# cleinc/bts

Measured on NVIDIA H100. Metric: training images/sec (352x704, DenseNet-161), higher is better.
Workload: dtype f32

## Files before the change

bts_b200/_lib.py:

```python
import ctypes
import glob
import os
import subprocess

_HERE = os.path.dirname(os.path.abspath(__file__))
_ROOT = os.path.dirname(_HERE)
LIB_PATH = os.path.join(_HERE, "libbts_b200.so")
CSRC = os.path.join(_HERE, "csrc")

NVCC_FLAGS = ["-gencode", "arch=compute_90a,code=sm_90a", "-lineinfo", "-O3", "-std=c++17",
              "-Xcompiler", "-fPIC", "--expt-relaxed-constexpr"]


def sources():
    return sorted(glob.glob(os.path.join(CSRC, "*.cu")))


def needs_build():
    if not os.path.isfile(LIB_PATH):
        return True
    t = os.path.getmtime(LIB_PATH)
    deps = sources() + glob.glob(os.path.join(CSRC, "*.cuh")) + glob.glob(os.path.join(_ROOT, "include", "*.h"))
    return any(os.path.getmtime(f) > t for f in deps)

# ... 29 lines not shown
_ll = ctypes.c_longlong

SIGNATURES = {
    "bts_version": [ctypes.c_char_p, _i],
    "bts_lpg_fwd": [_p, _p, _i, _i, _i, _i, _i, _p],
    "bts_lpg_fwd_fused": [_p, _p, _p, _p, _f, _i, _i, _i, _i, _i, _i, _p],
    "bts_lpg_bwd": [_p, _p, _p, _i, _i, _i, _i, _i, _i, _p],
    "bts_lpg_bwd_fused": [_p, _p, _p, _f, _i, _p, _p, _i, _i, _i, _i, _i, _i, _p],
    "bts_lpg_fwd_h": [_p, _p, _i, _i, _i, _i, _i],
    "bts_lpg_bwd_h": [_p, _p, _p, _i, _i, _i, _i, _i, _i],
    "bts_silog_fwd": [_p, _p, _p, _ll, _f, _p, _p, _p],
    "bts_silog_bwd": [_p, _p, _p, _ll, _f, _p, _p, _p, _p],
    "bts_plane_head_fwd": [_p, _p, _p, _p, _f, _i, _i, _i, _i, _i, _p],
    "bts_plane_head_bwd": [_p, _p, _p, _p, _f, _i, _i, _i, _i, _i, _p],
    "bts_conv_n_tile": [_i],
    "bts_conv_packed_floats": [_i, _i, _i, _i],
    "bts_conv_pack_weights": [_p, _ll, _ll, _ll, _ll, _i, _i, _i, _i, _i, _p, _p],
    "bts_conv_fwd": [_p, _ll, _i, _i, _i, _i, _i, _i, _i, _i, _i, _i, _p, _i, _p, _p, _i, _p, _ll, _i, _i, _p],
    "bts_conv_fwd_stats": [_p, _ll, _i, _i, _i, _i, _i, _i, _i, _i, _i, _i, _p, _i, _p, _p, _i, _p, _ll, _i, _i, _p, _p, _p],
    "bts_conv_fwd_ex": [_p, _ll, _i, _i, _i, _i, _i, _i, _i, _i, _i, _i, _i, _i, _i, _p, _i, _p, _p, _i, _p, _ll, _i, _i, _p,
                        _p, _p],
    "bts_conv_fwd_bnbwd": [_p, _ll, _i, _i, _i, _i, _i, _i, _i, _i, _i, _i, _i, _i, _i, _p, _i, _p, _ll, _i, _p, _ll, _p, _i,
                           _p, _p, _p],
    "bts_bn_bwd_coef": [_p, _p, _ll, _i, _p, _p, _p, _p, _p],
    "bts_conv_group_window": [_i, _i],
    "bts_conv_packed_floats_grouped": [_i, _i, _i, _i],
    "bts_conv_group_n_tile": [_i],
    "bts_conv_pack_weights_grouped": [_p, _ll, _ll, _ll, _ll, _i, _i, _i, _i, _i, _p, _p],
    "bts_conv_wgrad_grouped_plan": [_i, _i, _i, _i, _i, _i, _i, _p, _p],
    "bts_conv_wgrad_grouped": [_p, _ll, _i, _i, _i, _i, _i, _i, _i, _i, _i, _i, _p, _ll, _p, _i, _p, _ll, _ll, _ll, _ll, _i, _p],
    "bts_conv_wgrad_plan": [_i, _i, _i, _i, _i, _i, _i, _i, _p, _p],
    "bts_conv_wgrad": [_p, _ll, _i, _i, _i, _i, _i, _i, _i, _i, _i, _i, _p, _p, _i, _p, _ll, _i, _p, _i, _p, _ll, _ll,
                       _ll, _ll, _i, _p],
    "bts_conv_c1_workspace_floats": [_i, _i],
    "bts_conv_c1_fwd": [_p, _ll, _i, _i, _i, _i, _i, _p, _ll, _ll, _ll, _i, _p, _p],
    "bts_conv_c1_dgrad": [_p, _p, _i, _i, _i, _i, _i, _p, _ll, _ll, _ll, _p, _ll, _p],
    "bts_conv_c1_wgrad": [_p, _ll, _p, _p, _i, _i, _i, _i, _i, _p, _p, _ll, _ll, _ll, _p],
    "bts_bn_stats": [_p, _ll, _ll, _i, _p, _p, _p],
    "bts_bn_finalize": [_p, _p, _ll, _i, _p, _p, _f, _f, _p, _p, _p, _p, _p, _p, _p],
    "bts_bn_finalize_track": [_p, _p, _ll, _i, _p, _p, _f, _f, _p, _p, _p, _p, _p, _p, _p, _p],
    "bts_bn_fold": [_i, _p, _p, _f, _p, _p, _p, _p, _p, _p, _p],
    "bts_bn_relu_bwd_reduce": [_p, _ll, _p, _ll, _ll, _i, _p, _p, _p, _p, _p, _p, _p, _p],
    "bts_bn_relu_bwd_apply": [_p, _ll, _p, _ll, _ll, _i, _p, _p, _p, _p, _ll, _i, _p],
    "bts_wgrad2_set_tma": [_i],
    "bts_wgrad2_set_min_pixels": [_ll],
    "bts_wgrad2_set_min_kblocks": [_i],
# ... 68 lines not shown
```

bts_b200/conv.py:

```python
import ctypes
import weakref

import torch

from . import _lib
from .ops import _need_cuda, _ptr, _stream

ACT = {None: 0, "none": 0, "elu": 1, "sigmoid": 2}
import os as _os

PW_FWD = _os.environ.get("BTS_B200_PW_FWD", "1") == "1"
PW_WGRAD = True
PW_MIN_PIXELS = 200000
TRACE = _os.environ.get("BTS_B200_TRACE", "0") == "1"
trace_log = []


def set_trace(on):
    global TRACE
    TRACE = bool(on)
    del trace_log[:]


SYNC_DEBUG = _os.environ.get("BTS_B200_SYNC", "0") == "1"
# ... 115 lines not shown
                                               _ptr(packed), _stream()), "bts_conv_pack_weights")
    _lib.count()
    _pack_cache[key] = (weakref.ref(weight), weight._version, w.data_ptr(), packed, int(groups))
    if len(_pack_cache) > 4096:
        for k in [k for k, v in _pack_cache.items() if v[0]() is None]:
            del _pack_cache[k]
    return packed


def _nhwc_view(x):
    B, C, H, W = x.shape
    sb, sc, sh, sw = x.stride()
    ok = (sc == 1 or C == 1) and sh == W * sw and sb == H * sh and sw >= C
    if not ok:
        x = x.contiguous(memory_format=torch.channels_last)
        sb, sc, sh, sw = x.stride()
        if C == 1:
            sw = 1
    return x, sw


def conv2d_tc(x, weight, stride=1, padding=0, dilation=1, pre_scale=None, pre_shift=None, pre_relu=False,
              upsample2=False, act=None, out=None, precision=0, packed=None, cout=None, transpose_flip=False,
              stats=None, groups=1, zero_stuff_out=None, bn_bwd=None):
    _need_cuda(x, weight)
    if x.dtype != torch.float32:
        raise TypeError("conv2d_tc computes in fp32 (3xTF32 on wgmma); got %s" % x.dtype)
    x, xs = _nhwc_view(x)
    B, Cin, Hs, Ws = x.shape
    Co, Ci, KH, KW = weight.shape
    kwin = 0
    if groups > 1:
        kwin = group_window(Co, Ci)
        if not kwin:
            raise ValueError("unsupported grouped conv %s" % (tuple(weight.shape),))
        Ci = Co
    elif transpose_flip:
        Co, Ci = Ci, Co
    if Ci != Cin:
        raise ValueError("weight expects %d input channels, got %d" % (Ci, Cin))
    if (PW_FWD and KH == 1 and KW == 1 and stride == 1 and padding == 0 and groups == 1 and not upsample2
            and zero_stuff_out is None and pre_scale is None and not pre_relu and stats is None and bn_bwd is None
            and precision == 0 and packed is None and act in ACT and B * Hs * Ws >= PW_MIN_PIXELS
            and xs % 4 == 0 and x.data_ptr() % 16 == 0 and _lib.lib().bts_conv_pw_fwd_eligible(Cin, Co)):
        if out is None:
            out = torch.empty((B, Co, Hs, Ws), device=x.device, dtype=torch.float32, memory_format=torch.channels_last)
            os_ = Co
# ... 20 lines not shown
        Hout, Wout = int(zero_stuff_out[0]), int(zero_stuff_out[1])
        if stride != 1 or upsample2:
            raise ValueError("zero_stuff_out needs stride 1 and no up-sample")
    else:
        mode = 1 if upsample2 else 0
        Hin, Win = (2 * Hs, 2 * Ws) if upsample2 else (Hs, Ws)
        Hout = (Hin + 2 * padding - dilation * (KH - 1) - 1) // stride + 1
        Wout = (Win + 2 * padding - dilation * (KW - 1) - 1) // stride + 1
    if out is None:
        out = torch.empty((B, Co, Hout, Wout), device=x.device, dtype=torch.float32,
                          memory_format=torch.channels_last)
        os_ = Co
    else:
        if tuple(out.shape) != (B, Co, Hout, Wout):
            raise ValueError("out has shape %s, expected %s" % (tuple(out.shape), (B, Co, Hout, Wout)))
        o2, os_ = _nhwc_view(out)
        if o2 is not out:
            raise ValueError("out must be NHWC in memory")
    if pre_scale is not None:
        pre_scale = pre_scale.contiguous()
        pre_shift = pre_shift.contiguous()
    if stats is not None and (stats.dtype != torch.float64 or tuple(stats.shape) != (2, Co) or not stats.is_contiguous()):
        raise ValueError("stats must be a contiguous fp64 [2, Cout] tensor")
    if bn_bwd is not None:
        xb, st, relu = bn_bwd
        xb, xbs = _nhwc_view(xb)
        if stats is None or act is not None or pre_scale is not None or pre_relu or tuple(xb.shape) != (B, Co, Hout, Wout) \
                or tuple(st.shape) != (4, Co) or not st.is_contiguous():
            raise ValueError("bn_bwd needs zeroed stats, no act / pre-op, x_bn shaped like the output and st = [4, Cout]")
        with torch.cuda.device(x.device):
            rc = _traced("dgrad" if transpose_flip else "fwd",
                         "%dx%dx%d %d->%d k%d d%d s%d%s bnb" % (B, Hs, Ws, Cin, Co, KH, dilation, stride, " zs" if mode == 2 else ""),
                         lambda: _lib.lib().bts_conv_fwd_bnbwd(_ptr(x), xs, B, Hs, Ws, mode, Hout if mode == 2 else 0,
                                                               Wout if mode == 2 else 0, kwin, Cin, KH, KW, stride, padding,
                                                               dilation, _ptr(packed), Co, _ptr(out), os_, int(precision),
                                                               _ptr(xb), xbs, _ptr(st), int(bool(relu)), _ptr(stats[0]),
                                                               _ptr(stats[1]), _stream()),
                         2.0 * B * Hout * Wout * Co * (Cin // groups) * KH * KW)
        _lib.check(rc, "bts_conv_fwd_bnbwd")
        _lib.count()
        return out
    with torch.cuda.device(x.device):
        call = lambda: _lib.lib().bts_conv_fwd_ex(_ptr(x), xs, B, Hs, Ws, mode, Hout if mode == 2 else 0,
                                                  Wout if mode == 2 else 0, kwin, Cin, KH, KW, stride, padding, dilation,
                                                  _ptr(packed), Co, _ptr(pre_scale), _ptr(pre_shift), int(pre_relu),
                                                  _ptr(out), os_, ACT[act], int(precision),
                                                  _ptr(stats[0]) if stats is not None else None,
                                                  _ptr(stats[1]) if stats is not None else None, _stream())
        rc = _traced("dgrad" if transpose_flip else "fwd",
                     "%dx%dx%d %d->%d k%d d%d s%d%s%s" % (B, Hs, Ws, Cin, Co, KH, dilation, stride,
                                                         " up" if upsample2 else (" zs" if mode == 2 else ""),
                                                         " g%d" % groups if groups > 1 else ""),
                     call, 2.0 * B * Hout * Wout * Co * (Cin // groups) * KH * KW / (4.0 if mode == 2 else 1.0))
    _lib.check(rc, "bts_conv_fwd_ex")
    _lib.count()
    return out


def wgrad_grouped_tc(x, gy, weight_shape, weight_strides, stride=1, padding=0, dilation=1, precision=0):
    _need_cuda(x, gy)
    x, xs = _nhwc_view(x)
    gy, gs = _nhwc_view(gy)
    B, width, Hs, Ws = x.shape
    _, cpg, KH, KW = weight_shape
    L = _lib.lib()
    split = ctypes.c_int(0)
    wsf = ctypes.c_longlong(0)
    _lib.check(L.bts_conv_wgrad_grouped_plan(B, gy.shape[2], gy.shape[3], width, cpg, KH, KW, ctypes.byref(split),
                                             ctypes.byref(wsf)), "bts_conv_wgrad_grouped_plan")
    ws = torch.empty(wsf.value, device=x.device, dtype=torch.float32)
    gw = torch.empty_strided(tuple(weight_shape), tuple(weight_strides), device=x.device, dtype=torch.float32)
    s = weight_strides
    with torch.cuda.device(x.device):
        rc = _traced("wgrad", "%dx%dx%d %d->%d k%d d%d s%d g%d" % (B, Hs, Ws, width, width, KH, dilation, stride, width // cpg),
                     lambda: L.bts_conv_wgrad_grouped(_ptr(x), xs, B, Hs, Ws, width, cpg, KH, KW, stride, padding, dilation,
                                                      _ptr(gy), gs, _ptr(ws), split.value, _ptr(gw), s[0], s[1], s[2], s[3],
                                                      int(precision), _stream()),
# ... 148 lines not shown
```

bts_b200/csrc/conv_tc.cu:

```cuda
#include <cstdio>
#include <cstdlib>
#include <type_traits>

#include "tc_common.cuh"

namespace {

constexpr int BLOCK_M = 128;
constexpr int BLOCK_K = 32;
constexpr int MAX_N = 128;
constexpr int A_TILE_BYTES = BLOCK_M * 128;
constexpr int CONSUMER_THREADS = 256;
constexpr int PRODUCER_THREADS = 128;
constexpr int NUM_THREADS = CONSUMER_THREADS + 2 * PRODUCER_THREADS;
constexpr int PRODUCER_REGS = 80;
constexpr int CONSUMER_REGS = 176;
static_assert(CONSUMER_THREADS * CONSUMER_REGS + 2 * PRODUCER_THREADS * PRODUCER_REGS <= NUM_THREADS * 128,
              "the reallocation must fit the registers the CTA was launched with");
constexpr int MAX_CIN_SMEM = 4096;

struct ConvParams {
    const float *x;
    long long xs;
    int B, Hs, Ws;
// ... 469 lines not shown
            case 32: consume(std::integral_constant<int, 32>()); break;
            case 48: consume(std::integral_constant<int, 48>()); break;
            case 64: consume(std::integral_constant<int, 64>()); break;
            case 80: consume(std::integral_constant<int, 80>()); break;
            case 96: consume(std::integral_constant<int, 96>()); break;
            case 112: consume(std::integral_constant<int, 112>()); break;
            default: consume(std::integral_constant<int, 128>()); break;
        }
        if (p.stat_sum && p.n_tiles == 1) {
            asm volatile("bar.sync 1, %0;" ::"n"(CONSUMER_THREADS) : "memory");
            for (int c = (int)threadIdx.x; c < p.Cout; c += CONSUMER_THREADS) {
                double t1 = 0.0, t2 = 0.0;
                for (int w = 0; w < STAT_SETS; ++w) {
                    t1 += s_stat[(size_t)w * 2 * n_tile + c];
                    t2 += s_stat[(size_t)w * 2 * n_tile + n_tile + c];
                }
                atomicAdd(p.stat_sum + c, t1);
                atomicAdd(p.stat_sumsq + c, t2);
            }
        }
    }
}


}

extern "C" int bts_conv_n_tile(int Cout) {
    int n = (Cout + 15) / 16 * 16;
    if (n > MAX_N) {
        const int tiles = (n + MAX_N - 1) / MAX_N;
        n = ((Cout + tiles - 1) / tiles + 15) / 16 * 16;
    }
    return n;
}

extern "C" long long bts_conv_packed_floats(int n_rows, int k_channels, int KH, int KW) {
    const int n_tile = bts_conv_n_tile(n_rows);
    const int n_tiles = (n_rows + n_tile - 1) / n_tile;
    const int CQ = (k_channels + 3) / 4;
    const int KB = (KH * KW * CQ + 7) / 8;
    return (long long)n_tiles * KB * 2 * n_tile * 32;
}

extern "C" int bts_conv_pack_weights(const float *w, long long s_co, long long s_ci, long long s_kh, long long s_kw,
                                     int Cout, int Cin, int KH, int KW, int transpose_flip, float *wpack, void *stream) {
    if (!w || !wpack || Cout < 1 || Cin < 1 || KH < 1 || KW < 1) return BTS_EINVAL;
// ... 40 lines not shown

extern "C" int bts_conv_pack_weights_grouped(const float *w, long long s_co, long long s_ci, long long s_kh, long long s_kw,
                                             int width, int cpg, int KH, int KW, int transpose_flip, float *wpack,
                                             void *stream) {
    if (!w || !wpack || KH < 1 || KW < 1) return BTS_EINVAL;
    const int kwin = bts_conv_group_window(width, cpg);
    if (!kwin) return BTS_EINVAL;
    if (!bts_aligned16(wpack)) return BTS_EALIGN;
    const long long total = bts_conv_packed_floats_grouped(width, cpg, KH, KW) / 2;
    long long grid = (total + 255) / 256;
    const long long cap = (long long)bts_num_sms() * 16;
    if (grid > cap) grid = cap;
    pack_weights_kernel<<<(int)grid, 256, 0, (cudaStream_t)stream>>>(w, s_co, s_ci, s_kh, s_kw, width, width, KH, KW,
                                                                    transpose_flip, wpack, bts_conv_group_n_tile(kwin),
                                                                    width / bts_conv_group_n_tile(kwin), kwin, cpg);
    BTS_LAUNCH_CHECK();
    return 0;
}

struct BnBwdArgs {
    const float *x; long long xs; const float *st; int relu;
};

static int conv_fwd_impl(const float *x, long long x_pixel_stride, int B, int Hs, int Ws, int upsample2, int out_h,
                         int out_w, int kwin, int Cin,
                         int KH, int KW, int stride, int pad, int dil, const float *wpack, int Cout,
                         const float *pre_scale, const float *pre_shift, int pre_relu, float *out,
                         long long out_pixel_stride, int act, int precision, double *stat_sum, double *stat_sumsq,
                         void *stream, const BnBwdArgs *bnb = nullptr) {
    if (!x || !wpack || !out || B < 0 || Hs < 1 || Ws < 1 || Cin < 1 || Cout < 1 || KH < 1 || KW < 1 || stride < 1 ||
        pad < 0 || dil < 1)
        return BTS_EINVAL;
    if ((pre_scale == nullptr) != (pre_shift == nullptr)) return BTS_EINVAL;
    if (pre_scale && Cin > MAX_CIN_SMEM) return BTS_EINVAL;
    if (act < 0 || act > 2 || precision < 0 || precision > 1) return BTS_EINVAL;
    if (upsample2 < 0 || upsample2 > 2 || kwin < 0) return BTS_EINVAL;
    if (upsample2 == 2 && (stride != 1 || out_h < 1 || out_w < 1)) return BTS_EINVAL;
    if (kwin && (pre_scale || Cin % kwin || Cout % kwin)) return BTS_EINVAL;
    if (!bts_aligned16(wpack)) return BTS_EALIGN;
    if (B == 0) return 0;
    if ((long long)B * Hs * Ws * x_pixel_stride >= 0x7fffffffLL) return BTS_EINVAL;
    ConvParams p;
    p.x = x; p.xs = x_pixel_stride; p.B = B; p.Hs = Hs; p.Ws = Ws; p.up = upsample2; p.Cin = kwin ? kwin : Cin;
    p.kwin = kwin;
    p.KH = KH; p.KW = KW; p.stride = stride; p.pad = pad; p.dil = dil;
    p.wpack = wpack; p.Cout = Cout;
    if (kwin % 16) return BTS_EINVAL;
    p.n_tile = kwin ? bts_conv_group_n_tile(kwin) : bts_conv_n_tile(Cout);
    p.n_tiles = (Cout + p.n_tile - 1) / p.n_tile;
    p.pre_scale = pre_scale; p.pre_shift = pre_shift; p.pre_relu = pre_relu ? 1 : 0;
    p.out = out; p.os = out_pixel_stride; p.act = act; p.precision = precision;
    p.stat_sum = stat_sum; p.stat_sumsq = stat_sumsq;
// ... 7 lines not shown
    const int Hin = p.up ? 2 * Hs : Hs, Win = p.up ? 2 * Ws : Ws;
    p.Hv = Hin; p.Wv = Win;
    p.Hout = p.up == 2 ? out_h : (Hin + 2 * pad - dil * (KH - 1) - 1) / stride + 1;
    p.Wout = p.up == 2 ? out_w : (Win + 2 * pad - dil * (KW - 1) - 1) / stride + 1;
    if (p.Hout < 1 || p.Wout < 1) return BTS_EINVAL;
    if (Hin >= 0x4000 || Win >= 0x4000 || p.Hout >= 0x4000 || p.Wout >= 0x4000 || pad >= 0x4000 ||
        dil * (KH - 1) >= 0x4000 || dil * (KW - 1) >= 0x4000)
        return BTS_EINVAL;
    p.M = (long long)B * p.Hout * p.Wout;
    p.KC = (p.Cin + 31) / 32;
    p.CQ = (p.Cin + 3) / 4;
    p.KB = (KH * KW * p.CQ + 7) / 8;
    p.fd_cq = make_fastdiv((uint32_t)p.CQ);
    p.fd_kw = make_fastdiv((uint32_t)KW);
    p.vec_ok = bts_aligned16(x) && (x_pixel_stride % 4 == 0);
    const long long m_tiles = (p.M + BLOCK_M - 1) / BLOCK_M;
    if (m_tiles * p.n_tiles * (long long)p.KB > 0x7fffffffLL || p.M + BLOCK_M >= 0x7fffffffLL) return BTS_EINVAL;
    p.m_tiles = (int)m_tiles;
    p.total_tiles = (int)(m_tiles * p.n_tiles);
    p.fd_wout = make_fastdiv((uint32_t)p.Wout);
    p.fd_hout = make_fastdiv((uint32_t)p.Hout);
    p.fd_ntiles = make_fastdiv((uint32_t)p.n_tiles);
    const int pre = (pre_scale ? 2 : 0) | (p.pre_relu ? 1 : 0);
    p.stage_bytes = A_TILE_BYTES + 2 * p.n_tile * 128;
    const int pre_bytes = pre >= 2 ? p.KC * 32 * 8 : 0;
    const int stat_bytes = stat_sum ? STAT_SETS * 2 * p.n_tile * 8 : 0;
    p.stages = (SMEM_LIMIT - 1024 - BAR_BYTES - pre_bytes - stat_bytes) / p.stage_bytes;
    if (p.stages > MAX_STAGES) p.stages = MAX_STAGES;
    if (p.stages < 2) return BTS_EINVAL;
    const int smem = p.stages * p.stage_bytes + pre_bytes + BAR_BYTES + stat_bytes + 1024;
    const int sms = bts_num_sms();
    dim3 grid((unsigned)(p.total_tiles < sms ? p.total_tiles : sms));
    const bool vec = p.vec_ok;
    cudaError_t err = cudaSuccess;
#define BTS_LAUNCH(PRE, UP, VEC)                                                                                   \
    do {                                                                                                           \
        static bool attr_set_[BTS_MAX_DEVICES] = {};                                                               \
        bool &attr_set = attr_set_[bts_cur_device()];                                                              \
        if (!attr_set) {                                                                                           \
            err = cudaFuncSetAttribute(conv_tc_kernel<PRE, UP, VEC>, cudaFuncAttributeMaxDynamicSharedMemorySize,  \
                                       SMEM_LIMIT);                                                                \
            if (err != cudaSuccess) return (int)err;                                                               \
            attr_set = true;                                                                                       \
        }                                                                                                          \
        conv_tc_kernel<PRE, UP, VEC><<<grid, NUM_THREADS, smem, (cudaStream_t)stream>>>(p);                        \
    } while (0)
#define BTS_DISPATCH_UV(PRE)                                                                                       \
    do {                                                                                                           \
        if (p.up == 2) { if (vec) BTS_LAUNCH(PRE, 2, true); else BTS_LAUNCH(PRE, 2, false); }                      \
        else if (p.up) { if (vec) BTS_LAUNCH(PRE, 1, true); else BTS_LAUNCH(PRE, 1, false); }                      \
        else { if (vec) BTS_LAUNCH(PRE, 0, true); else BTS_LAUNCH(PRE, 0, false); }                                \
    } while (0)
    switch (pre) {
        case 0: BTS_DISPATCH_UV(0); break;
// ... 34 lines not shown
                         Cout, pre_scale, pre_shift, pre_relu, out, out_pixel_stride, act, precision, stat_sum, stat_sumsq,
                         stream);
}

extern "C" int bts_conv_pack_weights_multi(const void *descs, int n, long long total, void *stream) {
    if (!descs || n < 1 || total < 1) return BTS_EINVAL;
    long long grid = (total + 255) / 256;
    const long long cap = (long long)bts_num_sms() * 16;
    if (grid > cap) grid = cap;
    pack_weights_multi_kernel<<<(int)grid, 256, 0, (cudaStream_t)stream>>>(reinterpret_cast<const PackDesc *>(descs), n, total);
    BTS_LAUNCH_CHECK();
    return 0;
}

extern "C" int bts_conv_fwd_bnbwd(const float *x, long long x_pixel_stride, int B, int Hs, int Ws, int source_mode, int out_h,
                                  int out_w, int kwin, int Cin, int KH, int KW, int stride, int pad, int dil,
                                  const float *wpack, int Cout, float *out, long long out_pixel_stride, int precision,
                                  const float *x_bn, long long x_bn_stride, const float *bn_st, int relu, double *S1,
                                  double *S2, void *stream) {
    BnBwdArgs a{x_bn, x_bn_stride, bn_st, relu};
    return conv_fwd_impl(x, x_pixel_stride, B, Hs, Ws, source_mode, out_h, out_w, kwin, Cin, KH, KW, stride, pad, dil, wpack,
                         Cout, nullptr, nullptr, 0, out, out_pixel_stride, 0, precision, S1, S2, stream, &a);
}
```

include/bts_b200.h:

```cpp
#ifndef BTS_B200_H_
#define BTS_B200_H_

#include <stddef.h>
#include <stdint.h>

#ifdef __cplusplus
extern "C" {
#endif

#define BTS_LAYOUT_NCHW 0
#define BTS_LAYOUT_NHWC 1

#define BTS_EINVAL (-1)
#define BTS_EALIGN (-2)

int bts_version(char *buf, int buflen);

int bts_lpg_fwd(const float *plane, float *depth, int B, int h, int w, int r, int layout, void *stream);
int bts_lpg_fwd_fused(const float *plane, float *depth, float *scaled, float *ds, float max_depth,
                      int ds_stride, int B, int h, int w, int r, int layout, void *stream);

int bts_lpg_bwd(const float *dy, const float *plane, float *dplane, int B, int h, int w, int r,
                int layout, int tf_compat, void *stream);
int bts_lpg_bwd_fused(const float *d_depth, const float *d_scaled, const float *d_ds, float max_depth,
// ... 22 lines not shown
                 int KH, int KW, int stride, int pad, int dil, const float *wpack, int Cout,
                 const float *pre_scale, const float *pre_shift, int pre_relu, float *out,
                 long long out_pixel_stride, int act, int precision, void *stream);

int bts_conv_fwd_stats(const float *x, long long x_pixel_stride, int B, int Hs, int Ws, int upsample2, int Cin,
                       int KH, int KW, int stride, int pad, int dil, const float *wpack, int Cout,
                       const float *pre_scale, const float *pre_shift, int pre_relu, float *out,
                       long long out_pixel_stride, int act, int precision, double *stat_sum, double *stat_sumsq,
                       void *stream);

int bts_conv_fwd_ex(const float *x, long long x_pixel_stride, int B, int Hs, int Ws, int source_mode, int out_h, int out_w,
                    int kwin, int Cin, int KH, int KW, int stride, int pad, int dil, const float *wpack, int Cout,
                    const float *pre_scale, const float *pre_shift, int pre_relu, float *out, long long out_pixel_stride,
                    int act, int precision, double *stat_sum, double *stat_sumsq, void *stream);
int bts_wgrad2_set_tma(int on);
int bts_wgrad2_set_min_pixels(long long n);
int bts_wgrad2_set_min_kblocks(int n);
int bts_wgrad2_set_pointwise(int on);

int bts_conv_fwd_bnbwd(const float *x, long long x_pixel_stride, int B, int Hs, int Ws, int source_mode, int out_h, int out_w,
                       int kwin, int Cin, int KH, int KW, int stride, int pad, int dil, const float *wpack, int Cout,
                       float *out, long long out_pixel_stride, int precision, const float *x_bn, long long x_bn_stride,
                       const float *bn_st, int relu, double *S1, double *S2, void *stream);
int bts_bn_bwd_coef(const double *S1, const double *S2, long long M, int C, const float *scale, const float *mean,
                    const float *invstd, float *coef, void *stream);
int bts_conv_group_window(int width, int cpg);
int bts_conv_group_n_tile(int kwin);
long long bts_conv_packed_floats_grouped(int width, int cpg, int KH, int KW);
int bts_conv_pack_weights_grouped(const float *w, long long s_co, long long s_ci, long long s_kh, long long s_kw, int width,
                                  int cpg, int KH, int KW, int transpose_flip, float *wpack, void *stream);
int bts_conv_wgrad_grouped_plan(int B, int Hout, int Wout, int width, int cpg, int KH, int KW, int *splitK_out,
                                long long *workspace_floats);
int bts_conv_wgrad_grouped(const float *x, long long x_pixel_stride, int B, int Hs, int Ws, int width, int cpg, int KH, int KW,
                           int stride, int pad, int dil, const float *dy, long long dy_pixel_stride, float *workspace,
                           int splitK, float *dw, long long s_co, long long s_ci, long long s_kh, long long s_kw,
                           int precision, void *stream);

int bts_conv_wgrad_plan(int B, int Hout, int Wout, int Cin, int Cout, int KH, int KW, int stride, int *splitK_out,
                        long long *workspace_floats);
int bts_conv_wgrad(const float *x, long long x_pixel_stride, int B, int Hs, int Ws, int upsample2, int Cin,
                   int KH, int KW, int stride, int pad, int dil, const float *pre_scale, const float *pre_shift,
                   int pre_relu, const float *dy, long long dy_pixel_stride, int Cout, float *workspace, int splitK,
                   float *dw, long long s_co, long long s_ci, long long s_kh, long long s_kw, int precision,
                   void *stream);

int bts_conv_c1_workspace_floats(int C, int K);
// ... 89 lines not shown
```

Baseline: 82.13.

## Add halo-tiled implicit-GEMM conv forward kernel with automatic routing

Adds a warp-specialized conv kernel that loads a 2D spatial output tile plus its halo into shared memory once per channel chunk, then reuses it across all 3x3 taps. Previously each tap's A tile was staged separately. The input pre-op (affine/ReLU) is applied in shared memory by the fill threads. A new route entry point picks the halo path by default when its plan fits and the tile count per SM is no worse. The trade-offs are extra shared memory, which cuts the weight pipeline depth, and padding waste on partial spatial tiles.

```diff
diff --git a/bts_b200/_lib.py b/bts_b200/_lib.py
--- a/bts_b200/_lib.py
+++ b/bts_b200/_lib.py
@@ -75,6 +75,8 @@
                         _p, _p],
     "bts_conv_fwd_bnbwd": [_p, _ll, _i, _i, _i, _i, _i, _i, _i, _i, _i, _i, _i, _i, _i, _p, _i, _p, _ll, _i, _p, _ll, _p, _i,
                            _p, _p, _p],
+    "bts_conv_fwd_route": [_p, _ll, _i, _i, _i, _i, _i, _i, _i, _i, _i, _i, _i, _i, _i, _p, _i, _p, _p, _i, _p, _ll, _i, _i,
+                           _p, _p, _p, _ll, _p, _i, _i, _p],
     "bts_bn_bwd_coef": [_p, _p, _ll, _i, _p, _p, _p, _p, _p],
     "bts_conv_group_window": [_i, _i],
     "bts_conv_packed_floats_grouped": [_i, _i, _i, _i],
diff --git a/bts_b200/conv.py b/bts_b200/conv.py
--- a/bts_b200/conv.py
+++ b/bts_b200/conv.py
@@ -161,7 +161,7 @@
 
 def conv2d_tc(x, weight, stride=1, padding=0, dilation=1, pre_scale=None, pre_shift=None, pre_relu=False,
               upsample2=False, act=None, out=None, precision=0, packed=None, cout=None, transpose_flip=False,
-              stats=None, groups=1, zero_stuff_out=None, bn_bwd=None):
+              stats=None, groups=1, zero_stuff_out=None, bn_bwd=None, route=0):
     _need_cuda(x, weight)
     if x.dtype != torch.float32:
         raise TypeError("conv2d_tc computes in fp32 (3xTF32 on wgmma); got %s" % x.dtype)
@@ -228,37 +228,28 @@
         pre_shift = pre_shift.contiguous()
     if stats is not None and (stats.dtype != torch.float64 or tuple(stats.shape) != (2, Co) or not stats.is_contiguous()):
         raise ValueError("stats must be a contiguous fp64 [2, Cout] tensor")
+    xb, xbs, st, relu = None, 0, None, False
     if bn_bwd is not None:
         xb, st, relu = bn_bwd
         xb, xbs = _nhwc_view(xb)
         if stats is None or act is not None or pre_scale is not None or pre_relu or tuple(xb.shape) != (B, Co, Hout, Wout) \
                 or tuple(st.shape) != (4, Co) or not st.is_contiguous():
             raise ValueError("bn_bwd needs zeroed stats, no act / pre-op, x_bn shaped like the output and st = [4, Cout]")
-        with torch.cuda.device(x.device):
-            rc = _traced("dgrad" if transpose_flip else "fwd",
-                         "%dx%dx%d %d->%d k%d d%d s%d%s bnb" % (B, Hs, Ws, Cin, Co, KH, dilation, stride, " zs" if mode == 2 else ""),
-                         lambda: _lib.lib().bts_conv_fwd_bnbwd(_ptr(x), xs, B, Hs, Ws, mode, Hout if mode == 2 else 0,
-                                                               Wout if mode == 2 else 0, kwin, Cin, KH, KW, stride, padding,
-                                                               dilation, _ptr(packed), Co, _ptr(out), os_, int(precision),
-                                                               _ptr(xb), xbs, _ptr(st), int(bool(relu)), _ptr(stats[0]),
-                                                               _ptr(stats[1]), _stream()),
-                         2.0 * B * Hout * Wout * Co * (Cin // groups) * KH * KW)
-        _lib.check(rc, "bts_conv_fwd_bnbwd")
-        _lib.count()
-        return out
     with torch.cuda.device(x.device):
-        call = lambda: _lib.lib().bts_conv_fwd_ex(_ptr(x), xs, B, Hs, Ws, mode, Hout if mode == 2 else 0,
-                                                  Wout if mode == 2 else 0, kwin, Cin, KH, KW, stride, padding, dilation,
-                                                  _ptr(packed), Co, _ptr(pre_scale), _ptr(pre_shift), int(pre_relu),
-                                                  _ptr(out), os_, ACT[act], int(precision),
-                                                  _ptr(stats[0]) if stats is not None else None,
-                                                  _ptr(stats[1]) if stats is not None else None, _stream())
+        call = lambda: _lib.lib().bts_conv_fwd_route(_ptr(x), xs, B, Hs, Ws, mode, Hout if mode == 2 else 0,
+                                                     Wout if mode == 2 else 0, kwin, Cin, KH, KW, stride, padding, dilation,
+                                                     _ptr(packed), Co, _ptr(pre_scale), _ptr(pre_shift), int(pre_relu),
+                                                     _ptr(out), os_, ACT[act], int(precision),
+                                                     _ptr(stats[0]) if stats is not None else None,
+                                                     _ptr(stats[1]) if stats is not None else None,
+                                                     _ptr(xb), xbs, _ptr(st), int(bool(relu)), int(route), _stream())
         rc = _traced("dgrad" if transpose_flip else "fwd",
-                     "%dx%dx%d %d->%d k%d d%d s%d%s%s" % (B, Hs, Ws, Cin, Co, KH, dilation, stride,
-                                                         " up" if upsample2 else (" zs" if mode == 2 else ""),
-                                                         " g%d" % groups if groups > 1 else ""),
-                     call, 2.0 * B * Hout * Wout * Co * (Cin // groups) * KH * KW / (4.0 if mode == 2 else 1.0))
-    _lib.check(rc, "bts_conv_fwd_ex")
+                     "%dx%dx%d %d->%d k%d d%d s%d%s%s%s" % (B, Hs, Ws, Cin, Co, KH, dilation, stride,
+                                                           " up" if upsample2 else (" zs" if mode == 2 else ""),
+                                                           " g%d" % groups if groups > 1 else "",
+                                                           " bnb" if bn_bwd is not None else ""),
+                     call, 2.0 * B * Hout * Wout * Co * (Cin // groups) * KH * KW / (4.0 if mode == 2 and bn_bwd is None else 1.0))
+    _lib.check(rc, "bts_conv_fwd_route")
     _lib.count()
     return out
 
diff --git a/bts_b200/csrc/conv_tc.cu b/bts_b200/csrc/conv_tc.cu
--- a/bts_b200/csrc/conv_tc.cu
+++ b/bts_b200/csrc/conv_tc.cu
@@ -515,6 +515,405 @@
     }
 }
 
+constexpr int HALO_FILL_THREADS = 224;
+constexpr int HALO_MAX_KC = 8;
+constexpr int HALO_MAX_BSTAGES = 8;
+constexpr int HALO_BAR_BYTES = 512;
+constexpr int HALO_MAX_ITEMS = 8;
+
+struct HaloParams {
+    ConvParams c;
+    int TH, TW, tw_shift;
+    int hw, hpix;
+    int nwx, nwy;
+    FastDiv fd_nwx, fd_nwy, fd_hw;
+    int nh;
+    int chunk_bytes;
+    int bstages, bstage_bytes;
+};
+
+template <int PRE, int UP>
+__global__ void __launch_bounds__(NUM_THREADS, 1) conv_halo_kernel(const HaloParams h) {
+    const ConvParams &p = h.c;
+    extern __shared__ __align__(1024) uint8_t smem_raw[];
+    const uint32_t base = (smem_u32(smem_raw) + 1023u) & ~1023u;
+    uint8_t *sm = smem_raw + (base - smem_u32(smem_raw));
+    const int KC = p.KC, KB = p.KB, NH = h.nh, S = h.bstages;
+    const uint32_t chunk_bytes = (uint32_t)h.chunk_bytes, halo_bytes = (uint32_t)KC * chunk_bytes;
+    const uint32_t b_off = (uint32_t)NH * halo_bytes;
+    const uint32_t bstage_bytes = (uint32_t)h.bstage_bytes;
+    const uint32_t pre_off = b_off + (uint32_t)S * bstage_bytes;
+    float *s_scale = reinterpret_cast<float *>(sm + pre_off);
+    float *s_shift = s_scale + KC * 32;
+    const uint32_t bar_off = pre_off + (PRE >= 2 ? (uint32_t)KC * 32u * 8u : 0u);
+    const uint32_t bar0 = base + bar_off;
+    auto hfull = [&](int i) { return bar0 + 8u * i; };
+    auto hempty = [&](int i) { return bar0 + 8u * (2 * HALO_MAX_KC + i); };
+    auto bfull = [&](int s) { return bar0 + 8u * (4 * HALO_MAX_KC + s); };
+    auto bempty = [&](int s) { return bar0 + 8u * (4 * HALO_MAX_KC + HALO_MAX_BSTAGES + s); };
+    double *s_stat = reinterpret_cast<double *>(sm + bar_off + HALO_BAR_BYTES);
+
+    const int warp = threadIdx.x >> 5, lane = threadIdx.x & 31;
+    const int n_tile = p.n_tile;
+    if (p.stat_sum)
+        for (int i = threadIdx.x; i < STAT_SETS * 2 * n_tile; i += NUM_THREADS) s_stat[i] = 0.0;
+    const int my_tiles = (p.total_tiles - (int)blockIdx.x + (int)gridDim.x - 1) / (int)gridDim.x;
+
+    if (threadIdx.x == 0) {
+        for (int i = 0; i < NH * KC; ++i) {
+            mbar_init(hfull(i), HALO_FILL_THREADS);
+            mbar_init(hempty(i), CONSUMER_THREADS / 32);
+        }
+        for (int s = 0; s < S; ++s) {
+            mbar_init(bfull(s), 1);
+            mbar_init(bempty(s), CONSUMER_THREADS / 32);
+        }
+        asm volatile("fence.mbarrier_init.release.cluster;" ::: "memory");
+    }
+    if (PRE >= 2) {
+        for (int c = threadIdx.x; c < KC * 32; c += NUM_THREADS) {
+            s_scale[c] = p.pre_scale[c];
+            s_shift[c] = p.pre_shift[c];
+        }
+    }
+    __syncthreads();
+
+    auto window = [&](int tile, int &b, int &y0, int &x0, int &nt) {
+        const uint32_t m_tile = fdiv((uint32_t)tile, p.fd_ntiles);
+        nt = tile - (int)m_tile * p.n_tiles;
+        const uint32_t q = fdiv(m_tile, h.fd_nwx);
+        const uint32_t bb = fdiv(q, h.fd_nwy);
+        x0 = (int)(m_tile - q * (uint32_t)h.nwx) * h.TW;
+        y0 = (int)(q - bb * (uint32_t)h.nwy) * h.TH;
+        b = (int)bb;
+    };
+
+    if (threadIdx.x >= CONSUMER_THREADS) {
+        setmaxnreg_dec<PRODUCER_REGS>();
+        const int pt = threadIdx.x - CONSUMER_THREADS;
+        if (pt >= HALO_FILL_THREADS) {
+            if (pt != HALO_FILL_THREADS) return;
+            const uint32_t wbytes = 2u * (uint32_t)n_tile * 128u;
+            const uint8_t *wsrc = reinterpret_cast<const uint8_t *>(p.wpack);
+            int s = 0;
+            uint32_t ph = 0;
+#pragma unroll 1
+            for (int ti = 0; ti < my_tiles; ++ti) {
+                const int tile = (int)blockIdx.x + ti * (int)gridDim.x;
+                const int nt = tile - (int)fdiv((uint32_t)tile, p.fd_ntiles) * p.n_tiles;
+                const uint8_t *src = wsrc + (size_t)nt * KB * wbytes;
+#pragma unroll 1
+                for (int kb = 0; kb < KB; ++kb) {
+                    mbar_wait(bempty(s), ph ^ 1);
+                    mbar_arrive_expect_tx(bfull(s), wbytes);
+                    bulk_copy_g2s(base + b_off + (uint32_t)s * bstage_bytes, src + (size_t)kb * wbytes, wbytes, bfull(s));
+                    if (++s == S) { s = 0; ph ^= 1; }
+                }
+            }
+            return;
+        }
+        constexpr bool AFF = PRE >= 2;
+        constexpr bool RELU = (PRE & 1) != 0;
+        const int unit = pt & 7;
+        const int pix0 = pt >> 3;
+        const int items = (h.hpix - pix0 + HALO_FILL_THREADS / 8 - 1) / (HALO_FILL_THREADS / 8);
+        const int xs = (int)p.xs;
+        const int Hs = p.Hs, Ws = p.Ws;
+        const float *__restrict__ xg = p.x;
+        int img = 0, sy0 = 0, sx0 = 0;
+        uint32_t mask = 0;
+        auto item_off = [&](int j) {
+            const int px = pix0 + j * (HALO_FILL_THREADS / 8);
+            const int hy = (int)fdiv((uint32_t)px, h.fd_hw);
+            return ((img * Hs + sy0 + hy) * Ws + sx0 + px - hy * h.hw) * xs + unit * 4;
+        };
+        auto pre_op = [&](uint32_t dst_c, int c) {
+            float sc[4] = {1.f, 1.f, 1.f, 1.f}, sh[4] = {0.f, 0.f, 0.f, 0.f};
+            if (AFF) {
+                const float4 a4 = *reinterpret_cast<const float4 *>(s_scale + c * 32 + unit * 4);
+                const float4 b4 = *reinterpret_cast<const float4 *>(s_shift + c * 32 + unit * 4);
+                sc[0] = a4.x; sc[1] = a4.y; sc[2] = a4.z; sc[3] = a4.w;
+                sh[0] = b4.x; sh[1] = b4.y; sh[2] = b4.z; sh[3] = b4.w;
+            }
+#pragma unroll
+            for (int j = 0; j < HALO_MAX_ITEMS; ++j) {
+                if (!((mask >> j) & 1u)) continue;
+                const int px = pix0 + j * (HALO_FILL_THREADS / 8);
+                const uint32_t a = dst_c + (uint32_t)px * 128u + (uint32_t)((unit ^ (px & 7)) << 4);
+                const float4 q4 = ld_shared_v4(a);
+                float v[4] = {q4.x, q4.y, q4.z, q4.w};
+#pragma unroll
+                for (int e = 0; e < 4; ++e) {
+                    float x = v[e];
+                    if (AFF) x = fmaf(x, sc[e], sh[e]);
+                    if (RELU) x = fmaxf(x, 0.f);
+                    v[e] = x;
+                }
+                st_shared_v4(a, v[0], v[1], v[2], v[3]);
+            }
+        };
+        int pend_c = -1;
+        uint32_t pend_dst = 0, pend_bar = 0;
+        auto publish_pending = [&]() {
+            pre_op(pend_dst, pend_c);
+            mbar_arrive(pend_bar);
+        };
+#pragma unroll 1
+        for (int ti = 0; ti < my_tiles; ++ti) {
+            int b, y0, x0, nt;
+            window((int)blockIdx.x + ti * (int)gridDim.x, b, y0, x0, nt);
+            img = b;
+            sy0 = UP ? (y0 - p.pad) >> 1 : y0 - p.pad;
+            sx0 = UP ? (x0 - p.pad) >> 1 : x0 - p.pad;
+            mask = 0;
+#pragma unroll
+            for (int j = 0; j < HALO_MAX_ITEMS; ++j) {
+                const int px = pix0 + j * (HALO_FILL_THREADS / 8);
+                const int hy = (int)fdiv((uint32_t)px, h.fd_hw);
+                const int sy = sy0 + hy, sx = sx0 + px - hy * h.hw;
+                const bool ok = j < items && (unsigned)sy < (unsigned)Hs && (unsigned)sx < (unsigned)Ws;
+                mask |= (ok ? 1u : 0u) << j;
+            }
+            const int hb = NH == 1 ? 0 : (ti & 1);
+            const uint32_t hph = (uint32_t)(NH == 1 ? ti : ti >> 1) & 1u;
+            const uint32_t halo = base + (uint32_t)hb * halo_bytes;
+#pragma unroll 1
+            for (int c = 0; c < KC; ++c) {
+                const uint32_t dst_c = halo + (uint32_t)c * chunk_bytes;
+                const uint32_t bar = hfull(hb * KC + c);
+                mbar_wait(hempty(hb * KC + c), hph ^ 1);
+#pragma unroll
+                for (int j = 0; j < HALO_MAX_ITEMS; ++j) {
+                    if (j < items) {
+                        const int px = pix0 + j * (HALO_FILL_THREADS / 8);
+                        const bool ok = (mask >> j) & 1u;
+                        cp_async16(dst_c + (uint32_t)px * 128u + (uint32_t)((unit ^ (px & 7)) << 4),
+                                   ok ? xg + item_off(j) + c * 32 : xg, ok ? 16u : 0u);
+                    }
+                }
+                if constexpr (PRE == 0) {
+                    cp_async_mbar_arrive(bar);
+                } else {
+                    cp_async_commit();
+                    if (pend_c >= 0) {
+                        cp_async_wait_dyn(1);
+                        publish_pending();
+                    }
+                    pend_c = c; pend_dst = dst_c; pend_bar = bar;
+                }
+            }
+            if (PRE != 0) {
+                cp_async_wait_dyn(0);
+                publish_pending();
+                pend_c = -1;
+            }
+        }
+    } else {
+        setmaxnreg_inc<CONSUMER_REGS>();
+        const int wg = warp >> 2;
+        const int row = wg * 64 + (warp & 3) * 16 + (lane >> 2);
+        const bool single = p.precision != 0;
+        const int e = UP ? (p.pad & 1) : 0;
+        const uint32_t rc = (uint32_t)((row >> h.tw_shift) + e) | ((uint32_t)((row & (h.TW - 1)) + e) << 8) |
+                            ((uint32_t)(((row + 8) >> h.tw_shift) + e) << 16) |
+                            ((uint32_t)(((row + 8) & (h.TW - 1)) + e) << 24);
+        auto consume = [&](auto NT) {
+            constexpr int N = decltype(NT)::value;
+            constexpr int R = N / 2;
+            float acc[R], tot[R];
+            const uint64_t oBlo = (uint64_t)((N * 128) >> 4);
+            const uint32_t q4 = (threadIdx.x & 3u) * 4u;
+            int s = 0;
+            uint32_t ph = 0;
+            for (int ti = 0; ti < my_tiles; ++ti) {
+                const int hb = NH == 1 ? 0 : (ti & 1);
+                const uint32_t hph = (uint32_t)(NH == 1 ? ti : ti >> 1) & 1u;
+                const uint32_t halo = base + (uint32_t)hb * halo_bytes;
+#pragma unroll
+                for (int i = 0; i < R; ++i) tot[i] = 0.f;
+                int c = 0, tap = 0;
+                for (int kb = 0; kb < KB; ++kb) {
+                    if (tap == 0) mbar_wait_no_trap(hfull(hb * KC + c), hph);
+                    mbar_wait_no_trap(bfull(s), ph);
+                    const int ky = (tap * 11) >> 5, kx = tap - 3 * ky;
+                    auto hpix = [&](int sh) {
+                        const int ry = (int)((rc >> sh) & 0xffu) + ky, rx = (int)((rc >> (sh + 8)) & 0xffu) + kx;
+                        return UP ? (ry >> 1) * h.hw + (rx >> 1) : ry * h.hw + rx;
+                    };
+                    const int hp0 = hpix(0), hp1 = hpix(16);
+                    const uint32_t hc = halo + (uint32_t)c * chunk_bytes + q4;
+                    const uint32_t a0 = hc + (uint32_t)hp0 * 128u + ((uint32_t)(hp0 & 7) << 4);
+                    const uint32_t a1 = hc + (uint32_t)hp1 * 128u + ((uint32_t)(hp1 & 7) << 4);
+                    uint32_t hi[BLOCK_K / 8][4], lo[BLOCK_K / 8][4];
+#pragma unroll
+                    for (int k = 0; k < BLOCK_K / 8; ++k) {
+#pragma unroll
+                        for (int j = 0; j < 4; ++j) {
+                            const uint32_t x = ld_shared_u32(((j & 1) ? a1 : a0) ^ (uint32_t)(32 * k + 16 * (j >> 1)));
+                            float hh, ll;
+                            split_tf32(__uint_as_float(x), hh, ll);
+                            hi[k][j] = __float_as_uint(hh);
+                            lo[k][j] = __float_as_uint(ll);
+                        }
+                    }
+                    const uint64_t d = make_desc(base + b_off + (uint32_t)s * bstage_bytes);
+                    wgmma_fence();
+                    if (single) {
+#pragma unroll
+                        for (int k = 0; k < BLOCK_K / 8; ++k) Wgmma<N>::mma_rs(acc, hi[k], d + 2 * k, k != 0);
+                    } else {
+#pragma unroll
+                        for (int k = 0; k < BLOCK_K / 8; ++k) {
+                            const uint64_t dbh = d + 2 * k, dbl = dbh + oBlo;
+                            Wgmma<N>::mma_rs(acc, lo[k], dbh, k != 0);
+                            Wgmma<N>::mma_rs(acc, hi[k], dbl, 1);
+                            Wgmma<N>::mma_rs(acc, hi[k], dbh, 1);
+                        }
+                    }
+                    wgmma_commit();
+                    wgmma_wait<0>();
+                    wgmma_fence_operands(acc);
+#pragma unroll
+                    for (int k = 0; k < BLOCK_K / 8; ++k) {
+                        wgmma_fence_operands(hi[k]);
+                        wgmma_fence_operands(lo[k]);
+                    }
+                    __syncwarp();
+                    if (lane == 0) {
+                        mbar_arrive(bempty(s));
+                        if (tap == 8) mbar_arrive(hempty(hb * KC + c));
+                    }
+#pragma unroll
+                    for (int i = 0; i < R; ++i) tot[i] += acc[i];
+                    if (++s == S) { s = 0; ph ^= 1; }
+                    if (++c == KC) { c = 0; ++tap; }
+                }
+
+                int cq = ((int)threadIdx.x & 3) * 2, Cout = p.Cout, pe = UP ? p.pad & 1 : 0;
+                const float *bnb_x = p.bnb_x, *bnb_st = p.bnb_st;
+                asm volatile("" : "+r"(cq), "+r"(Cout), "+r"(pe), "+l"(bnb_x), "+l"(bnb_st));
+                int b, y0, x0, nt;
+                window((int)blockIdx.x + ti * (int)gridDim.x, b, y0, x0, nt);
+                const int ty0 = (int)(rc & 0xffu) - pe, tx0 = (int)((rc >> 8) & 0xffu) - pe;
+                const int ty1 = (int)((rc >> 16) & 0xffu) - pe, tx1 = (int)(rc >> 24) - pe;
+                const bool v0 = y0 + ty0 < p.Hout && x0 + tx0 < p.Wout;
+                const bool v1 = y0 + ty1 < p.Hout && x0 + tx1 < p.Wout;
+                const int m0 = v0 ? (b * p.Hout + y0 + ty0) * p.Wout + x0 + tx0 : 0;
+                const int m1 = v1 ? (b * p.Hout + y0 + ty1) * p.Wout + x0 + tx1 : 0;
+                const bool ovec = ((p.os & 1) == 0) && ((((uintptr_t)p.out) & 7) == 0);
+                float *orow0 = p.out + (long long)m0 * p.os + (long long)nt * n_tile;
+                float *orow1 = p.out + (long long)m1 * p.os + (long long)nt * n_tile;
+#pragma unroll
+                for (int j = 0; j < N / 8; ++j) {
+                    const int col = 8 * j + cq;
+                    const int cabs = nt * n_tile + col;
+#pragma unroll
+                    for (int i = 0; i < 2; ++i) {
+                        float o[2];
+#pragma unroll
+                        for (int cc = 0; cc < 2; ++cc) {
+                            float a = tot[4 * j + 2 * i + cc];
+                            if (p.act == 1) a = a > 0.f ? a : expm1f(a);
+                            else if (p.act == 2) a = 1.0f / (1.0f + expf(-a));
+                            o[cc] = a;
+                        }
+                        if (i ? v1 : v0) {
+                            float *orow = i ? orow1 : orow0;
+                            if (ovec && cabs + 1 < Cout) {
+                                *reinterpret_cast<float2 *>(orow + col) = make_float2(o[0], o[1]);
+                            } else {
+                                if (cabs < Cout) orow[col] = o[0];
+                                if (cabs + 1 < Cout) orow[col + 1] = o[1];
+                            }
+                        }
+                    }
+                }
+                if (p.stat_sum) {
+#pragma unroll
+                    for (int j = 0; j < N / 8; ++j) {
+                        const int col = 8 * j + cq;
+                        const int cabs = nt * n_tile + col;
+#pragma unroll
+                        for (int cc = 0; cc < 2; ++cc) {
+                            float s1 = 0.f, s2 = 0.f;
+                            const int ch = cabs + cc;
+#pragma unroll
+                            for (int i = 0; i < 2; ++i) {
+                                const long long m = i ? m1 : m0;
+                                if ((i ? v1 : v0) && ch < Cout) {
+                                    const float g = tot[4 * j + 2 * i + cc];
+                                    if (bnb_x) {
+                                        const float xv = __ldg(bnb_x + m * p.bnb_xs + ch);
+                                        const float sc = __ldg(bnb_st + ch), sh = __ldg(bnb_st + Cout + ch);
+                                        const float mu = __ldg(bnb_st + 2 * Cout + ch), is = __ldg(bnb_st + 3 * Cout + ch);
+                                        const float y = fmaf(xv, sc, sh);
+                                        const float gm = (!p.bnb_relu || y > 0.f) ? g : 0.f;
+                                        s1 += gm;
+                                        s2 += gm * ((xv - mu) * is);
+                                    } else {
+                                        s1 += g;
+                                        s2 += g * g;
+                                    }
+                                }
+                            }
+#pragma unroll
+                            for (int w = 4; w <= 16; w <<= 1) {
+                                s1 += __shfl_xor_sync(0xffffffffu, s1, w);
+                                s2 += __shfl_xor_sync(0xffffffffu, s2, w);
+                            }
+                            if (lane < 4 && ch < Cout) {
+                                double *mine = s_stat + (size_t)warp * 2 * n_tile;
+                                mine[col + cc] += (double)s1;
+                                mine[n_tile + col + cc] += (double)s2;
+                            }
+                        }
+                    }
+                }
+                if (p.stat_sum && p.n_tiles > 1) {
+                    asm volatile("bar.sync 1, %0;" ::"n"(CONSUMER_THREADS) : "memory");
+                    for (int cc = (int)threadIdx.x; cc < n_tile; cc += CONSUMER_THREADS) {
+                        const int ch = nt * n_tile + cc;
+                        double t1 = 0.0, t2 = 0.0;
+                        for (int w = 0; w < STAT_SETS; ++w) {
+                            t1 += s_stat[(size_t)w * 2 * n_tile + cc];
+                            t2 += s_stat[(size_t)w * 2 * n_tile + n_tile + cc];
+                            s_stat[(size_t)w * 2 * n_tile + cc] = 0.0;
+                            s_stat[(size_t)w * 2 * n_tile + n_tile + cc] = 0.0;
+                        }
+                        if (ch < p.Cout) {
+                            atomicAdd(p.stat_sum + ch, t1);
+                            atomicAdd(p.stat_sumsq + ch, t2);
+                        }
+                    }
+                    asm volatile("bar.sync 1, %0;" ::"n"(CONSUMER_THREADS) : "memory");
+                }
+            }
+        };
+        switch (n_tile) {
+            case 16: consume(std::integral_constant<int, 16>()); break;
+            case 32: consume(std::integral_constant<int, 32>()); break;
+            case 48: consume(std::integral_constant<int, 48>()); break;
+            case 64: consume(std::integral_constant<int, 64>()); break;
+            case 80: consume(std::integral_constant<int, 80>()); break;
+            case 96: consume(std::integral_constant<int, 96>()); break;
+            case 112: consume(std::integral_constant<int, 112>()); break;
+            default: consume(std::integral_constant<int, 128>()); break;
+        }
+        if (p.stat_sum && p.n_tiles == 1) {
+            asm volatile("bar.sync 1, %0;" ::"n"(CONSUMER_THREADS) : "memory");
+            for (int c = (int)threadIdx.x; c < p.Cout; c += CONSUMER_THREADS) {
+                double t1 = 0.0, t2 = 0.0;
+                for (int w = 0; w < STAT_SETS; ++w) {
+                    t1 += s_stat[(size_t)w * 2 * n_tile + c];
+                    t2 += s_stat[(size_t)w * 2 * n_tile + n_tile + c];
+                }
+                atomicAdd(p.stat_sum + c, t1);
+                atomicAdd(p.stat_sumsq + c, t2);
+            }
+        }
+    }
+}
+
 
 }
 
@@ -601,12 +1000,64 @@
     const float *x; long long xs; const float *st; int relu;
 };
 
+static bool halo_plan(const ConvParams &p, int pre, HaloParams &h) {
+    if (p.up > 1 || p.KH != 3 || p.KW != 3 || p.stride != 1 || p.dil != 1 || p.kwin || p.Cin % 32 || !p.vec_ok)
+        return false;
+    if (p.KC > HALO_MAX_KC) return false;
+    const bool stats = p.stat_sum != nullptr;
+    if (stats && p.Wout % 16) return false;
+    static const int shapes[3][2] = {{8, 16}, {16, 8}, {4, 32}};
+    long long best = -1;
+    int TH = 0, TW = 0;
+    for (const auto &s : shapes) {
+        if (stats && s[1] < 16) continue;
+        const long long area = (long long)((p.Hout + s[0] - 1) / s[0] * s[0]) * ((p.Wout + s[1] - 1) / s[1] * s[1]);
+        if (best < 0 || area < best) { best = area; TH = s[0]; TW = s[1]; }
+    }
+    h.c = p;
+    h.TH = TH; h.TW = TW;
+    h.tw_shift = TW == 8 ? 3 : TW == 16 ? 4 : 5;
+    const int hh = p.up ? TH / 2 + 2 : TH + 2;
+    h.hw = p.up ? TW / 2 + 2 : TW + 2;
+    h.hpix = hh * h.hw;
+    h.nwx = (p.Wout + TW - 1) / TW;
+    h.nwy = (p.Hout + TH - 1) / TH;
+    const long long m_tiles = (long long)p.B * h.nwx * h.nwy;
+    if (m_tiles * p.n_tiles * (long long)p.KB > 0x7fffffffLL) return false;
+    h.c.m_tiles = (int)m_tiles;
+    h.c.total_tiles = (int)(m_tiles * p.n_tiles);
+    h.fd_nwx = make_fastdiv((uint32_t)h.nwx);
+    h.fd_nwy = make_fastdiv((uint32_t)h.nwy);
+    h.fd_hw = make_fastdiv((uint32_t)h.hw);
+    h.chunk_bytes = (h.hpix * 128 + 1023) / 1024 * 1024;
+    h.bstage_bytes = 2 * p.n_tile * 128;
+    const int halo_bytes = p.KC * h.chunk_bytes;
+    const int fixed = 1024 + (pre >= 2 ? p.KC * 32 * 8 : 0) + HALO_BAR_BYTES + (stats ? STAT_SETS * 2 * p.n_tile * 8 : 0);
+    for (int nh = 2; nh >= 1; --nh) {
+        int st = (SMEM_LIMIT - fixed - nh * halo_bytes) / h.bstage_bytes;
+        if (st > HALO_MAX_BSTAGES) st = HALO_MAX_BSTAGES;
+        if (st >= 2) {
+            h.nh = nh;
+            h.bstages = st;
+            return true;
+        }
+    }
+    return false;
+}
+
+static int halo_smem_bytes(const HaloParams &h, int pre) {
+    const ConvParams &p = h.c;
+    return p.KC * h.chunk_bytes * h.nh + h.bstages * h.bstage_bytes + (pre >= 2 ? p.KC * 32 * 8 : 0) + HALO_BAR_BYTES +
+           (p.stat_sum ? STAT_SETS * 2 * p.n_tile * 8 : 0) + 1024;
+}
+
 static int conv_fwd_impl(const float *x, long long x_pixel_stride, int B, int Hs, int Ws, int upsample2, int out_h,
                          int out_w, int kwin, int Cin,
                          int KH, int KW, int stride, int pad, int dil, const float *wpack, int Cout,
                          const float *pre_scale, const float *pre_shift, int pre_relu, float *out,
                          long long out_pixel_stride, int act, int precision, double *stat_sum, double *stat_sumsq,
-                         void *stream, const BnBwdArgs *bnb = nullptr) {
+                         void *stream, const BnBwdArgs *bnb = nullptr, int route = 0) {
+    if (route < 0 || route > 2) return BTS_EINVAL;
     if (!x || !wpack || !out || B < 0 || Hs < 1 || Ws < 1 || Cin < 1 || Cout < 1 || KH < 1 || KW < 1 || stride < 1 ||
         pad < 0 || dil < 1)
         return BTS_EINVAL;
@@ -660,6 +1111,43 @@
     p.fd_hout = make_fastdiv((uint32_t)p.Hout);
     p.fd_ntiles = make_fastdiv((uint32_t)p.n_tiles);
     const int pre = (pre_scale ? 2 : 0) | (p.pre_relu ? 1 : 0);
+    const int sms = bts_num_sms();
+    if (route != 1) {
+        HaloParams h;
+        const bool ok = halo_plan(p, pre, h);
+        if (route == 2 && !ok) return BTS_EINVAL;
+        if (ok && (route == 2 || (h.c.total_tiles + sms - 1) / sms <= (p.total_tiles + sms - 1) / sms)) {
+            const int smem = halo_smem_bytes(h, pre);
+            dim3 grid((unsigned)(h.c.total_tiles < sms ? h.c.total_tiles : sms));
+            cudaError_t err = cudaSuccess;
+#define BTS_LAUNCH_HALO(PRE, UP)                                                                                   \
+    do {                                                                                                           \
+        static bool attr_set_[BTS_MAX_DEVICES] = {};                                                               \
+        bool &attr_set = attr_set_[bts_cur_device()];                                                              \
+        if (!attr_set) {                                                                                           \
+            err = cudaFuncSetAttribute(conv_halo_kernel<PRE, UP>, cudaFuncAttributeMaxDynamicSharedMemorySize,     \
+                                       SMEM_LIMIT);                                                                \
+            if (err != cudaSuccess) return (int)err;                                                               \
+            attr_set = true;                                                                                       \
+        }                                                                                                          \
+        conv_halo_kernel<PRE, UP><<<grid, NUM_THREADS, smem, (cudaStream_t)stream>>>(h);                           \
+    } while (0)
+#define BTS_DISPATCH_HALO(PRE)                                                                                     \
+    do {                                                                                                           \
+        if (p.up) BTS_LAUNCH_HALO(PRE, 1); else BTS_LAUNCH_HALO(PRE, 0);                                           \
+    } while (0)
+            switch (pre) {
+                case 0: BTS_DISPATCH_HALO(0); break;
+                case 1: BTS_DISPATCH_HALO(1); break;
+                case 2: BTS_DISPATCH_HALO(2); break;
+                default: BTS_DISPATCH_HALO(3); break;
+            }
+#undef BTS_DISPATCH_HALO
+#undef BTS_LAUNCH_HALO
+            BTS_LAUNCH_CHECK();
+            return 0;
+        }
+    }
     p.stage_bytes = A_TILE_BYTES + 2 * p.n_tile * 128;
     const int pre_bytes = pre >= 2 ? p.KC * 32 * 8 : 0;
     const int stat_bytes = stat_sum ? STAT_SETS * 2 * p.n_tile * 8 : 0;
@@ -667,7 +1155,6 @@
     if (p.stages > MAX_STAGES) p.stages = MAX_STAGES;
     if (p.stages < 2) return BTS_EINVAL;
     const int smem = p.stages * p.stage_bytes + pre_bytes + BAR_BYTES + stat_bytes + 1024;
-    const int sms = bts_num_sms();
     dim3 grid((unsigned)(p.total_tiles < sms ? p.total_tiles : sms));
     const bool vec = p.vec_ok;
     cudaError_t err = cudaSuccess;
@@ -748,3 +1235,15 @@
     return conv_fwd_impl(x, x_pixel_stride, B, Hs, Ws, source_mode, out_h, out_w, kwin, Cin, KH, KW, stride, pad, dil, wpack,
                          Cout, nullptr, nullptr, 0, out, out_pixel_stride, 0, precision, S1, S2, stream, &a);
 }
+
+extern "C" int bts_conv_fwd_route(const float *x, long long x_pixel_stride, int B, int Hs, int Ws, int source_mode, int out_h,
+                                  int out_w, int kwin, int Cin, int KH, int KW, int stride, int pad, int dil,
+                                  const float *wpack, int Cout, const float *pre_scale, const float *pre_shift, int pre_relu,
+                                  float *out, long long out_pixel_stride, int act, int precision, double *stat_sum,
+                                  double *stat_sumsq, const float *x_bn, long long x_bn_stride, const float *bn_st,
+                                  int bn_relu, int route, void *stream) {
+    BnBwdArgs a{x_bn, x_bn_stride, bn_st, bn_relu};
+    return conv_fwd_impl(x, x_pixel_stride, B, Hs, Ws, source_mode, out_h, out_w, kwin, Cin, KH, KW, stride, pad, dil, wpack,
+                         Cout, pre_scale, pre_shift, pre_relu, out, out_pixel_stride, act, precision, stat_sum, stat_sumsq,
+                         stream, x_bn ? &a : nullptr, route);
+}
diff --git a/include/bts_b200.h b/include/bts_b200.h
--- a/include/bts_b200.h
+++ b/include/bts_b200.h
@@ -68,6 +68,11 @@
                        int kwin, int Cin, int KH, int KW, int stride, int pad, int dil, const float *wpack, int Cout,
                        float *out, long long out_pixel_stride, int precision, const float *x_bn, long long x_bn_stride,
                        const float *bn_st, int relu, double *S1, double *S2, void *stream);
+int bts_conv_fwd_route(const float *x, long long x_pixel_stride, int B, int Hs, int Ws, int source_mode, int out_h, int out_w,
+                       int kwin, int Cin, int KH, int KW, int stride, int pad, int dil, const float *wpack, int Cout,
+                       const float *pre_scale, const float *pre_shift, int pre_relu, float *out, long long out_pixel_stride,
+                       int act, int precision, double *stat_sum, double *stat_sumsq, const float *x_bn,
+                       long long x_bn_stride, const float *bn_st, int bn_relu, int route, void *stream);
 int bts_bn_bwd_coef(const double *S1, const double *S2, long long M, int C, const float *scale, const float *mean,
                     const float *invstd, float *coef, void *stream);
 int bts_conv_group_window(int width, int cpg);
```

Result: no change. 82.84, median of 6 (+0.9%).
